# tsdconseil/libtsd

Measured on AMD Instinct MI355X. Metric: Msamples/s, 127-tap FIR on 2^26 cfloat stream, higher is better.
Workload: dtype f32 (complex64 data, real f32 taps); 1 GPU; configs[1]: 127-tap FIR (design_rif_fen lp 0.02, real taps via filtrer()) on 2^26-sample Veccf per GPU, inputs resident in HBM; method=overlap-save, samples_per_gpu=67108864, pre_warm_steps=150, backend=none (one process, one GPU), world_size=1, self_launched=False

## Files before the change

### libtsd_amd/csrc/ols.hip

```cpp
#include "fir_internal.hpp"
#include "fft1024_wave.hpp"
#include <cstdlib>

namespace tsdgpu {

using namespace w1024;
constexpr int OLS_N = 1024;
#ifndef OLS_SCALAR
#define OLS_SCALAR 1
#endif
#ifndef OLS_RUN_DEFAULT
#define OLS_RUN_DEFAULT 2
#endif
#ifndef OLS_DYN_DEFAULT
#define OLS_DYN_DEFAULT 16
#endif
constexpr int OLS_MAX_CTR = 32;
#if OLS_SCALAR
using cv = cpx;
#else
using cv = v2f;
#endif
__device__ __forceinline__ cv mkv(float a, float b) { return Make<cv>::of(a, b); }

constexpr bool NT = false;
__device__ __forceinline__ cv ntload(const cv *p)
{
  v2f t = __builtin_nontemporal_load(reinterpret_cast<const v2f *>(p));
  return mkv(t.x, t.y);
}
__device__ __forceinline__ void ntstore(cv *p, cv v)
{
  v2f t = {v.x, v.y};
  __builtin_nontemporal_store(t, reinterpret_cast<v2f *>(p));
}
template <bool EDGE>
__device__ __forceinline__ void ols_fetch_real(cv (&v)[16], const float *__restrict__ x, const float *__restrict__ hist,
                                               int histlen, int Km1, int L, int64_t n, int64_t b, int lane)
{
  const int64_t ga = 2 * b * (int64_t) L - Km1, gb = ga + L;
  if (!EDGE) {
    const float *xa = x + ga, *xb = x + gb;
#pragma unroll
    for (int r = 0; r < 16; r++) v[r] = mkv(xa[64 * r + lane], xb[64 * r + lane]);
  } else {
#pragma unroll
    for (int r = 0; r < 16; r++) {
      const int64_t g1 = ga + 64 * r + lane, g2 = gb + 64 * r + lane;
      v[r] = mkv(g1 < 0 ? hist[histlen + g1] : (g1 < n ? x[g1] : 0.f), g2 < 0 ? hist[histlen + g2] : (g2 < n ? x[g2] : 0.f));
    }
  }
}
template <bool EDGE>
__device__ __forceinline__ void ols_fetch(cv (&v)[16], const cv *__restrict__ x, const cv *__restrict__ hist,
                                          int histlen, int Km1, int L, int64_t n, int64_t b, int lane)
{
  const int64_t g0 = b * (int64_t) L - Km1;
  if (!EDGE) {
    const cv *xb = x + g0;
#pragma unroll
    for (int r = 0; r < 16; r++) v[r] = NT ? ntload(xb + 64 * r + lane) : xb[64 * r + lane];
  } else {
#pragma unroll
    for (int r = 0; r < 16; r++) {
      const int64_t g = g0 + 64 * r + lane;
      v[r] = g < 0 ? hist[histlen + g] : (g < n ? x[g] : mkv(0.f, 0.f));
    }
  }
}

struct OlsDyn {
  unsigned *ctr;
  unsigned base, Q;
  int NC;
  int64_t nunits;
};
struct RegTab {
  cv v[16];
  __device__ __forceinline__ const cv &operator[](int r) const { return v[r]; }
};

template <bool EDGE, bool REAL, int R0, bool DYN>
__device__ __forceinline__ void ols_body(cv *lds, const void *__restrict__ xv, const void *__restrict__ histv,
                                         void *__restrict__ yv, const cv *__restrict__ Hreg,
                                         const cv *__restrict__ TW1, const cv *__restrict__ TW2, int Km1,
                                         int histlen, int L, int64_t n, int64_t b_lo, int64_t b_hi, int64_t G,
                                         int64_t w, int64_t cgrp, int R, OlsDyn dyn)
{
  const int lane = threadIdx.x & 63;
  const cv *x = (const cv *) xv, *hist = (const cv *) histv;
  cv *y = (cv *) yv;
  const float *xr = (const float *) xv, *histr = (const float *) histv;
  float *yr = (float *) yv;
  RegTab tw1r, tw2r, Hr;
#pragma unroll
  for (int r = 0; r < 16; r++) {
    tw1r.v[r] = TW1[r * 64 + lane];
    tw2r.v[r] = TW2[r * 64 + lane];
    Hr.v[r] = Hreg[r * 64 + lane];
  }
  auto sync = []() {
    __builtin_amdgcn_fence(__ATOMIC_RELEASE, "wavefront");
    __builtin_amdgcn_wave_barrier();
    __builtin_amdgcn_fence(__ATOMIC_ACQUIRE, "wavefront");
  };

  const int64_t slot = (G % 8 == 0) ? (w % 8) * (G / 8) + w / 8 : w;
  const int ctr_c = DYN ? (int) (cgrp % dyn.NC) : 0;
  auto pull_issue = [&]() -> unsigned {
    unsigned v = 0;
    if (lane == 0) v = __hip_atomic_fetch_add(dyn.ctr + ctr_c * 32, 1u, __ATOMIC_RELAXED, __HIP_MEMORY_SCOPE_AGENT);
    return v;
  };
  auto pull = [&]() -> int64_t {
    for (;;) {
      const unsigned v = (unsigned) __builtin_amdgcn_readfirstlane((int) pull_issue()) - dyn.base;
      if (v >= dyn.Q) return -1;
      const int64_t u = (int64_t) v * dyn.NC + ctr_c;
      if (u < dyn.nunits) return u;
    }
  };
  auto pull_finish = [&](unsigned raw) -> int64_t {
    const unsigned v = (unsigned) __builtin_amdgcn_readfirstlane((int) raw) - dyn.base;
    if (v >= dyn.Q) return -1;
    const int64_t u = (int64_t) v * dyn.NC + ctr_c;
    return u < dyn.nunits ? u : pull();
  };
  int64_t unit = EDGE ? 0 : (DYN ? pull() : slot);
  if (unit < 0) return;
  int64_t run0 = EDGE ? b_lo : b_lo + unit * R;
  int64_t b = run0;
  if (b >= b_hi) return;

  int64_t pulled = -1;
  auto process = [&](cv (&cur)[16], cv (&nxt)[16], int64_t blk, int64_t nb, bool inrun) {
    const bool more = !EDGE && nb < b_hi;
    cv keep[R0 > 0 ? R0 : 1], pre[R0 > 0 ? R0 : 1];
#pragma unroll
    for (int r = 0; r < R0; r++) keep[r] = cur[(16 - R0 + r) & 15];
    const int64_t pb = more ? nb : blk;
    if (!EDGE && R0 > 0) {
      if (!REAL) {
        const cv *xb = x + (pb * (int64_t) L - Km1);
        if (!inrun) {
#pragma unroll
          for (int r = 0; r < R0; r++) pre[r] = xb[64 * r + lane];
        }
#pragma unroll
        for (int r = R0; r < 16; r++) nxt[r] = NT ? ntload(xb + 64 * r + lane) : xb[64 * r + lane];
      } else {
        const float *xa = xr + (2 * pb * (int64_t) L - Km1), *xb = xa + L;
        if (!inrun) {
#pragma unroll
          for (int r = 0; r < R0; r++) pre[r] = mkv(xa[64 * r + lane], xb[64 * r + lane]);
        }
#pragma unroll
        for (int r = R0; r < 16; r++) nxt[r] = mkv(xa[64 * r + lane], xb[64 * r + lane]);
      }
    } else if (!EDGE) {
      if (REAL) ols_fetch_real<EDGE>(nxt, xr, histr, histlen, Km1, L, n, pb, lane);
      else ols_fetch<EDGE>(nxt, x, hist, histlen, Km1, L, n, pb, lane);
    }
    const bool pulls = DYN && more && !inrun;
    unsigned raw = 0;
    if (pulls) raw = pull_issue();
    forward(cur, lds, lane, tw1r, tw2r, sync);
#pragma unroll
    for (int r = 0; r < 16; r++) cur[r] = cmul(cur[r], Hr[r]);
    inverse(cur, lds, lane, tw1r, tw2r, sync);
    sync();
    if (!EDGE) {
#pragma unroll
      for (int r = R0; r < 16; r++) asm volatile("" ::"v"(nxt[r]));
#pragma unroll
      for (int r = 0; r < R0; r++) {
        asm volatile("" : "+v"(keep[r]));
        if (inrun) nxt[r] = REAL ? mkv(keep[r].y, nxt[(16 - R0 + r) & 15].x) : keep[r];
        else nxt[r] = pre[r];
      }
    }
    if (pulls) pulled = pull_finish(raw);
    const int r0 = (!EDGE && R0 > 0) ? R0 : Km1 >> 6;
    if (!REAL) {
      const int64_t o0 = blk * (int64_t) L;
      cv *yb = y + (o0 - Km1);
#pragma unroll
      for (int r = 0; r < 16; r++) {
        const int t = 64 * r + lane;
        if (!EDGE) {
          if (r >= r0) { if (NT) ntstore(yb + t, cur[r]); else yb[t] = cur[r]; }
        } else {
          if (r >= r0 && o0 + t - Km1 < n) yb[t] = cur[r];
        }
      }
    } else {
      const int64_t oa = 2 * blk * (int64_t) L, ob = oa + L;
      float *ya = yr + (oa - Km1), *yb = yr + (ob - Km1);
#pragma unroll
      for (int r = 0; r < 16; r++) {
        const int t = 64 * r + lane;
        if (!EDGE) {
          if (r >= r0) { ya[t] = cur[r].x; yb[t] = cur[r].y; }
        } else {
          if (r >= r0 && oa + t - Km1 < n) ya[t] = cur[r].x;
          if (r >= r0 && ob + t - Km1 < n) yb[t] = cur[r].y;
        }
      }
    }
  };

  cv A[16], B[16];
  if (REAL) ols_fetch_real<EDGE>(A, xr, histr, histlen, Km1, L, n, b, lane);
  else ols_fetch<EDGE>(A, x, hist, histlen, Km1, L, n, b, lane);
  if (EDGE) {
    process(A, B, b, b_hi, false);
    return;
  }
#pragma unroll
  for (int r = 0; r < 16; r++) asm volatile("" ::"v"(A[r]));
  int i = 0;
  constexpr int64_t END = INT64_MAX;
  auto unit_after = [&](int64_t u) -> int64_t {
    if (DYN) return pulled;
    return b_lo + (u + G) * R < b_hi ? u + G : -1;
  };
  int64_t unit_next = DYN ? pull() : unit_after(unit);
  auto next_of = [&](int64_t &nb, bool &inrun) {
    inrun = i + 1 < R && b + 1 < b_hi;
    nb = inrun ? b + 1 : (unit_next >= 0 ? b_lo + unit_next * R : END);
  };
  auto advance = [&](int64_t nb, bool inrun) {
    if (inrun) i++;
    else {
      i = 0;
      run0 = nb;
      unit = unit_next;
      unit_next = unit_after(unit);
    }
    b = nb;
  };
  for (;;) {
    int64_t nb;
    bool inrun;
    next_of(nb, inrun);
    process(A, B, b, nb, inrun);
    if (nb >= b_hi) break;
    advance(nb, inrun);
    next_of(nb, inrun);
    process(B, A, b, nb, inrun);
    if (nb >= b_hi) break;
    advance(nb, inrun);
  }
}

template <bool REAL, int R0, bool DYN>
__global__ __launch_bounds__(64, 2) void ols_kernel(const void *__restrict__ x, const void *__restrict__ hist,
                                                    void *__restrict__ hist_next, void *__restrict__ y,
                                                    const cpx *__restrict__ Hreg, const cpx *__restrict__ TW1,
                                                    const cpx *__restrict__ TW2, int Km1, int histlen, int L,
                                                    int64_t n, int64_t b_lo, int64_t b_hi, int64_t nblocks, int G,
                                                    int ne, int64_t n_lo, int64_t b_tail, int R, OlsDyn dyn)
{
  __shared__ cv lds[LDS_ELEMS];
  const int64_t w = (int64_t) blockIdx.x;
  const int lane = threadIdx.x & 63;
  if (w < G) {
    ols_body<false, REAL, R0, DYN>(lds, x, hist, y, (const cv *) Hreg, (const cv *) TW1, (const cv *) TW2, Km1, histlen, L, n, b_lo, b_hi, G,
                                       w, (int64_t) blockIdx.x / 8, R, dyn);
  } else if (w < G + ne) {
    const int64_t b = (w - G) < n_lo ? (int64_t) (w - G) : b_tail + (w - G - n_lo);
    ols_body<true, REAL, 0, false>(lds, x, hist, y, (const cv *) Hreg, (const cv *) TW1, (const cv *) TW2, Km1, histlen, L, n, b, nblocks, 1, 0, 0, 1, dyn);
  } else if (w == G + ne) {
    for (int i = lane; i < histlen; i += 64) {
      const int64_t g = n - histlen + i;
      if (REAL) ((float *) hist_next)[i] = g < 0 ? ((const float *) hist)[histlen + g] : ((const float *) x)[g];
      else ((cpx *) hist_next)[i] = g < 0 ? ((const cpx *) hist)[histlen + g] : ((const cpx *) x)[g];
    }
  }
}

bool ols_preferred(const tsdgpu_fir *f)
{
  if (ols_long_supported(f)) return true;
  if (f->data_type == TSDGPU_C64) return f->K >= (f->tap_type == TSDGPU_F32 ? 57 : 48) && f->K <= 513;
  return f->tap_type == TSDGPU_F32 && f->K >= 40 && f->K <= 513;
}

int ols_plan_create(tsdgpu_fir *f)
{
  if (ols_long_supported(f)) return ols_long_plan_create(f);
  if (f->K > OLS_N - 63) {
    f->method = TSDGPU_FIR_DIRECT;
    return TSDGPU_OK;
  }
  const int N = OLS_N, K = f->K;
  f->ols_N = N;
  f->ols_L = N - (int) (cdiv(K - 1, 64) * 64);
  std::vector<double> hr(K), hi(K, 0.0);
  if (f->tap_type == TSDGPU_F32) {
    const float *t = (const float *) f->taps_host.data();
    for (int i = 0; i < K; i++) hr[i] = t[i];
  } else {
    const float *t = (const float *) f->taps_host.data();
    for (int i = 0; i < K; i++) { hr[i] = t[2 * i]; hi[i] = t[2 * i + 1]; }
  }
  struct Tables {
    std::vector<double> c, s;
    std::vector<cpx> tw12;
    Tables() : c(OLS_N / 2), s(OLS_N / 2), tw12(2 * OLS_N)
    {
      const double PI = 3.14159265358979323846;
      for (int i = 0; i < OLS_N / 2; i++) { c[i] = std::cos(2 * PI * i / OLS_N); s[i] = -std::sin(2 * PI * i / OLS_N); }
      fill_twiddles(tw12.data(), tw12.data() + OLS_N);
    }
  };
  static const Tables *tb = new Tables();
  std::vector<double> ar(N, 0.0), ai(N, 0.0);
  int logn = 0;
  while ((1 << logn) < N) logn++;
  for (int i = 0; i < K; i++) {
    int rv = 0;
    for (int b = 0; b < logn; b++) rv |= ((i >> b) & 1) << (logn - 1 - b);
    ar[rv] = hr[i];
    ai[rv] = hi[i];
  }
  for (int len = 2; len <= N; len <<= 1) {
    const int half = len / 2, step = N / len;
    for (int base = 0; base < N; base += len)
      for (int j = 0; j < half; j++) {
        const double wr = tb->c[(size_t) j * step], wi = tb->s[(size_t) j * step];
        const int a = base + j, b = a + half;
        const double tr = ar[b] * wr - ai[b] * wi, ti = ar[b] * wi + ai[b] * wr;
        ar[b] = ar[a] - tr; ai[b] = ai[a] - ti;
        ar[a] += tr; ai[a] += ti;
      }
  }
  std::vector<cpx> img(3 * (size_t) N);
  for (int lane = 0; lane < 64; lane++)
    for (int r = 0; r < 16; r++) {
      const int k = freq_index(lane, r);
      img[r * 64 + lane] = mk((float) (ar[k] / N), (float) (ai[k] / N));
    }
  std::copy(tb->tw12.begin(), tb->tw12.end(), img.begin() + N);
  const size_t bytes = (size_t) N * sizeof(cpx);
  const size_t ctr_bytes = (size_t) OLS_MAX_CTR * 128;
  img.resize(3 * (size_t) N + ctr_bytes / sizeof(cpx), mk(0.f, 0.f));
  if (hipMalloc(&f->d_H, 3 * bytes + ctr_bytes) != hipSuccess)
    return set_err(TSDGPU_ERR_HIP, "ols: hipMalloc failed: %s", hipGetErrorString(hipGetLastError()));
  if (hipMemcpy(f->d_H, img.data(), 3 * bytes + ctr_bytes, hipMemcpyHostToDevice) != hipSuccess)
    return set_err(TSDGPU_ERR_HIP, "ols: upload failed: %s", hipGetErrorString(hipGetLastError()));
  f->d_ctr = (unsigned *) ((char *) f->d_H + 3 * bytes);
  f->ctr_base = 0;
  static const std::pair<int, int> occ = []() {
    int dev = 0, cus = 256, per_cu = 8;
    (void) hipGetDevice(&dev);
    (void) hipDeviceGetAttribute(&cus, hipDeviceAttributeMultiprocessorCount, dev);
    if (hipOccupancyMaxActiveBlocksPerMultiprocessor(&per_cu, ols_kernel<false, 2, true>, 64, 0) != hipSuccess || per_cu < 1) {
      (void) hipGetLastError();
      per_cu = 8;
    }
    return std::make_pair(cus, per_cu);
  }();
  const int cus = occ.first, per_cu = occ.second;
  f->ols_grid = cus * per_cu;
  if (getenv("TSDGPU_DEBUG")) fprintf(stderr, "[tsdgpu] ols plan: N=%d K=%d L=%d cus=%d waves/CU=%d grid=%d waves\n", N, K, f->ols_L, cus, per_cu, f->ols_grid);
  return TSDGPU_OK;
}

void ols_plan_destroy(tsdgpu_fir *f)
{
  if (f->d_H) (void) hipFree(f->d_H);
  f->d_H = nullptr;
  f->d_ctr = nullptr;
}

int ols_step(tsdgpu_fir *f, const void *x, void *y, int64_t n, hipStream_t st)
{
  const bool real = f->data_type == TSDGPU_F32;
  const int L = f->ols_L;
  const int64_t LB = real ? 2 * (int64_t) L : L;
  const int64_t nblocks = cdiv(n, LB);
  const cpx *d = (const cpx *) f->d_H;
  const int64_t ovl = OLS_N - L;
  const int64_t b_lo = std::min<int64_t>(nblocks, f->K > 1 ? cdiv(ovl, LB) : 0);
  const int64_t b_hi = std::max<int64_t>(b_lo, n / LB);
  int64_t grid = 0;
  const int r0 = (int) (ovl / 64);
  const char *run_s = dev_switch("OLS_RUN");
  const int run_env = run_s ? atoi(run_s) : OLS_RUN_DEFAULT;
  const char *nc_s = dev_switch("OLS_DYN");
  int NC = nc_s ? atoi(nc_s) : OLS_DYN_DEFAULT;
  if (NC < 0 || NC > OLS_MAX_CTR || f->capturable || !f->d_ctr || stream_is_capturing(st)) NC = 0;
  int R = 1;
  unsigned ctr_add = 0;
  OlsDyn dyn = {f->d_ctr, f->ctr_base, 0u, NC > 0 ? NC : 1, 0};
  if (b_hi > b_lo) {
    const int64_t nint = b_hi - b_lo;
    if (r0 >= 1 && r0 <= 4 && run_env > 1 && nint >= (int64_t) f->ols_grid * run_env * 2) R = run_env;
    const int64_t nruns = cdiv(nint, R);
    const char *min_s = dev_switch("OLS_DYN_MIN");
    const int64_t dyn_min = min_s ? atoi(min_s) : 4;
    if (NC > 0 && nruns >= dyn_min * (int64_t) f->ols_grid) {
      const int64_t grp = (int64_t) 8 * NC;
      grid = std::max<int64_t>(grp, (f->ols_grid / grp) * grp);
      if (NC != f->ctr_nc) {
        TSD_HIP(hipMemsetAsync(f->d_ctr, 0, (size_t) OLS_MAX_CTR * 128, st));
        f->ctr_base = 0;
        f->ctr_nc = NC;
        dyn.base = 0;
      }
      dyn.nunits = nruns;
      dyn.Q = (unsigned) cdiv(nruns, NC);
      ctr_add = dyn.Q + (unsigned) (grid / NC);
    } else {
      NC = 0;
      grid = nruns < f->ols_grid ? nruns : f->ols_grid;
      if (nruns > grid) {
        const int64_t rounds = cdiv(nruns, grid);
        grid = cdiv(cdiv(nruns, rounds), 8) * 8;
      }
    }
  } else NC = 0;
  const int64_t b_lo_w = b_lo;
  const int64_t n_lo = b_lo, b_tail = b_hi;
  const int ne = (int) (n_lo + (nblocks - b_tail));
  int64_t e[2] = {n_lo, b_tail};
  const int nxt = f->cur ^ 1;
  const unsigned nwg = (unsigned) (grid + ne + 1);
#define OLS_LAUNCH(REAL, R0, DYN)                                                                                                     \
  hipLaunchKernelGGL((ols_kernel<REAL, R0, DYN>), dim3(nwg), dim3(64), 0, st, x, (const void *) fir_hist_read(f),                        \
                     f->hist[nxt], y, d, d + OLS_N, d + 2 * OLS_N, OLS_N - L, f->HL, L, n, b_lo_w, b_hi, nblocks, (int) grid, ne,   \
                     e[0], e[1], R, dyn)
#define OLS_LAUNCH_R0(REAL, DYN)                                        \
  switch (R > 1 ? r0 : 0) {                                             \
    case 1: OLS_LAUNCH(REAL, 1, DYN); break;                            \
    case 2: OLS_LAUNCH(REAL, 2, DYN); break;                            \
    case 3: OLS_LAUNCH(REAL, 3, DYN); break;                            \
    case 4: OLS_LAUNCH(REAL, 4, DYN); break;                            \
    default: OLS_LAUNCH(REAL, 0, DYN); break;                           \
  }
  if (real) {
    if (NC > 0) { OLS_LAUNCH_R0(true, true) } else { OLS_LAUNCH_R0(true, false) }
  } else {
    if (NC > 0) { OLS_LAUNCH_R0(false, true) } else { OLS_LAUNCH_R0(false, false) }
  }
#undef OLS_LAUNCH_R0
#undef OLS_LAUNCH
  if (const hipError_t le = hipGetLastError(); le != hipSuccess) {
    if (NC > 0) f->ctr_nc = 0;
    return set_err(TSDGPU_ERR_HIP, "fir_step: overlap-save launch failed: %s", hipGetErrorString(le));
  }
  f->ctr_base += ctr_add;
  f->cur = nxt;
  return TSDGPU_OK;
}

__global__ __launch_bounds__(64, 2) void ola1024_kernel(const cpx *__restrict__ x, cpx *__restrict__ y, const cpx *__restrict__ Hreg,
                                                        const cpx *__restrict__ TW1, const cpx *__restrict__ TW2,
                                                        const cpx *__restrict__ svg_in, cpx *__restrict__ svg_out, int64_t B, int per)
{
  __shared__ cv lds[LDS_ELEMS];
  const int lane = threadIdx.x;
  const int64_t b_lo = (int64_t) blockIdx.x * per, b_hi = min(B, b_lo + (int64_t) per);
  if (b_lo >= B) return;
  cv tw1[16], tw2[16], H[16];
#pragma unroll
  for (int r = 0; r < 16; r++) {
    tw1[r] = ((const cv *) TW1)[r * 64 + lane];
    tw2[r] = ((const cv *) TW2)[r * 64 + lane];
    H[r] = ((const cv *) Hreg)[r * 64 + lane];
  }
  auto sync = []() {
    __builtin_amdgcn_fence(__ATOMIC_RELEASE, "wavefront");
    __builtin_amdgcn_wave_barrier();
    __builtin_amdgcn_fence(__ATOMIC_ACQUIRE, "wavefront");
  };
  const cv *xs = (const cv *) x;
  cv *ys = (cv *) y;
  cv cur[16], carry[8], nxt[8];
  auto transform = [&](cv (&v)[16]) {
    forward(v, lds, lane, tw1, tw2, sync);
#pragma unroll
    for (int r = 0; r < 16; r++) v[r] = cmul(v[r], H[r]);
    inverse(v, lds, lane, tw1, tw2, sync);
    sync();
  };
  if (b_lo == 0) {
#pragma unroll
    for (int r = 0; r < 8; r++) carry[r] = ((const cv *) svg_in)[64 * r + lane];
  } else {
#pragma unroll
    for (int r = 0; r < 8; r++) { cur[r] = mkv(0.f, 0.f); cur[8 + r] = xs[(b_lo - 1) * 512 + 64 * r + lane]; }
    transform(cur);
#pragma unroll
    for (int r = 0; r < 8; r++) carry[r] = cur[8 + r];
  }
#pragma unroll
  for (int r = 0; r < 8; r++) nxt[r] = xs[b_lo * 512 + 64 * r + lane];
  for (int64_t b = b_lo; b < b_hi; b++) {
#pragma unroll
    for (int r = 0; r < 8; r++) { cur[r] = mkv(0.f, 0.f); cur[8 + r] = nxt[r]; }
    const bool more = b + 1 < b_hi;
    if (more) {
#pragma unroll
      for (int r = 0; r < 8; r++) nxt[r] = xs[(b + 1) * 512 + 64 * r + lane];
    }
    transform(cur);
    if (more) {
#pragma unroll
      for (int r = 0; r < 8; r++) asm volatile("" ::"v"(nxt[r]));
    }
#pragma unroll
    for (int r = 0; r < 8; r++) {
      ys[b * 512 + 64 * r + lane] = mkv(cur[r].x + carry[r].x, cur[r].y + carry[r].y);
      carry[r] = cur[8 + r];
    }
  }
  if (b_hi == B) {
#pragma unroll
    for (int r = 0; r < 8; r++) ((cv *) svg_out)[64 * r + lane] = carry[r];
  }
}

void ola1024_tables(const cpx *H_host, cpx *out3)
{
  for (int lane = 0; lane < 64; lane++)
    for (int r = 0; r < 16; r++) {
      const cpx h = H_host[freq_index(lane, r)];
      out3[r * 64 + lane] = mk(h.x / 1024.f, h.y / 1024.f);
    }
  fill_twiddles(out3 + 1024, out3 + 2048);
}

int ola1024_launch(const cpx *x, cpx *y, const cpx *tables3, const cpx *svg_in, cpx *svg_out, int64_t B, hipStream_t st)
{
  if (B <= 0) return TSDGPU_OK;
  const int per = (int) std::min<int64_t>(16, std::max<int64_t>(1, cdiv(B, 2048)));
  const int64_t grid = cdiv(B, per);
  if (grid > 0x7fffffff) return set_err(TSDGPU_ERR_UNSUPPORTED, "ola: too many blocks in one call");
  hipLaunchKernelGGL(ola1024_kernel, dim3((unsigned) grid), dim3(64), 0, st, x, y, tables3, tables3 + 1024, tables3 + 2048, svg_in, svg_out, B, per);
  TSD_HIP(hipGetLastError());
  return TSDGPU_OK;
}

__global__ __launch_bounds__(64, 2) void olaw512_kernel(const cpx *__restrict__ blk0, int nrest, const cpx *__restrict__ x, cpx *__restrict__ y,
                                                        const cpx *__restrict__ Hreg, const cpx *__restrict__ TW1, const cpx *__restrict__ TW2,
                                                        const float *__restrict__ fen, const cpx *__restrict__ svg_in,
                                                        const cpx *__restrict__ last_in, const cpx *__restrict__ prev_half_in,
                                                        cpx *__restrict__ svg_out, cpx *__restrict__ last_out, int64_t B, int per,
                                                        int skip_first)
{
  __shared__ cv lds[LDS_ELEMS];
  const int lane = threadIdx.x;
  const int64_t b_lo = (int64_t) blockIdx.x * per, b_hi = min(B, b_lo + (int64_t) per);
  if (b_lo >= B) return;
  const int sig = (lane >> 1) & 1, c = 2 * (lane >> 2) + (lane & 1);
  cv tw1[16], tw2[16], H[8];
  float win[16];
#pragma unroll
  for (int r = 0; r < 16; r++) {
    tw1[r] = ((const cv *) TW1)[r * 64 + lane];
    tw2[r] = ((const cv *) TW2)[r * 64 + lane];
    win[r] = fen[32 * r + c];
  }
#pragma unroll
  for (int q = 0; q < 8; q++) H[q] = ((const cv *) Hreg)[q * 64 + lane];
  auto sync = []() {
    __builtin_amdgcn_fence(__ATOMIC_RELEASE, "wavefront");
    __builtin_amdgcn_wave_barrier();
    __builtin_amdgcn_fence(__ATOMIC_ACQUIRE, "wavefront");
  };
  auto sample = [&](int64_t i) -> cv {
    if (i < 0) return ((const cv *) prev_half_in)[i + 256];
    if (i < 512) return ((const cv *) blk0)[i];
    return ((const cv *) x)[i - nrest];
  };
  auto xchg = [&](cv a) -> cv {
    return mkv(__shfl_xor(a.x, 2), __shfl_xor(a.y, 2));
  };
  cv v[16], keep[8];
  int64_t p = b_lo <= 1 ? 0 : b_lo - 2;
  if (b_lo <= 1) {
#pragma unroll
    for (int r = 0; r < 8; r++) keep[r] = ((const cv *) svg_in)[256 + 32 * r + c];
    if (b_lo == 0 && !skip_first) {
#pragma unroll
      for (int r = 0; r < 8; r++) {
        const int i = 32 * r + c;
        cv o = ((const cv *) last_in)[256 * sig + i];
        if (sig) {
          const cv g = ((const cv *) svg_in)[i];
          o = mkv(o.x + g.x * 0.5f, o.y + g.y * 0.5f);
        }
        ((cv *) y)[256 * sig + i] = o;
      }
    }
  } else {
#pragma unroll
    for (int r = 0; r < 8; r++) keep[r] = mkv(0.f, 0.f);
  }
  const int64_t p_end = b_hi == B ? B : b_hi - 1;
  for (; p < p_end; p++) {
    const int64_t base = 512 * p - 256 + 256 * sig;
#pragma unroll
    for (int r = 0; r < 16; r++) {
      const cv a = sample(base + 32 * r + c);
      v[r] = mkv(a.x * win[r], a.y * win[r]);
    }
    forward_pair512(v, lds, lane, tw1, tw2, sync);
#pragma unroll
    for (int r = 0; r < 16; r++) v[r] = cmul(v[r], H[2 * (r >> 2) + (r & 1)]);
    inverse_pair512(v, lds, lane, tw1, tw2, sync);
    sync();
    cv got[8];
#pragma unroll
    for (int r = 0; r < 8; r++) got[r] = xchg(v[8 + r]);
    if (p + 1 < B) {
      if (p + 1 >= b_lo) {
        cv *yo = (cv *) y + (p + 1 - skip_first) * 512 + 256 * sig + c;
#pragma unroll
        for (int r = 0; r < 8; r++) {
          const cv o = sig ? got[r] : keep[r];
          yo[32 * r] = mkv(o.x * 0.5f + v[r].x * 0.5f, o.y * 0.5f + v[r].y * 0.5f);
        }
      }
    } else {
      if (sig) {
#pragma unroll
        for (int r = 0; r < 16; r++) ((cv *) svg_out)[32 * r + c] = v[r];
      } else {
#pragma unroll
        for (int r = 0; r < 8; r++) {
          ((cv *) last_out)[32 * r + c] = mkv(keep[r].x * 0.5f + v[r].x * 0.5f, keep[r].y * 0.5f + v[r].y * 0.5f);
          ((cv *) last_out)[256 + 32 * r + c] = mkv(v[8 + r].x * 0.5f, v[8 + r].y * 0.5f);
        }
      }
    }
#pragma unroll
    for (int r = 0; r < 8; r++) keep[r] = got[r];
  }
}

void olaw512_tables(const cpx *H_host, cpx *out)
{
  for (int lane = 0; lane < 64; lane++)
    for (int q = 0; q < 8; q++) {
      const cpx h = H_host[pair512_freq_index(lane, 4 * (q >> 1) + (q & 1))];
      out[q * 64 + lane] = mk(h.x / 512.f, h.y / 512.f);
    }
  fill_twiddles_pair512(out + 512, out + 512 + 1024);
}

int olaw512_launch(const cpx *blk0, int nrest, const cpx *x, cpx *y, const cpx *tables, const float *fen, const cpx *svg_in, const cpx *last_in,
                   const cpx *prev_half_in, cpx *svg_out, cpx *last_out, int64_t B, int skip_first, hipStream_t st)
{
  if (B <= 0) return TSDGPU_OK;
  const int per = (int) std::min<int64_t>(16, std::max<int64_t>(2, cdiv(B, 2048)));
  const int64_t grid = cdiv(B, per);
  if (grid > 0x7fffffff) return set_err(TSDGPU_ERR_UNSUPPORTED, "ola: too many blocks in one call");
  hipLaunchKernelGGL(olaw512_kernel, dim3((unsigned) grid), dim3(64), 0, st, blk0, nrest, x, y, tables, tables + 512, tables + 512 + 1024, fen, svg_in,
                     last_in, prev_half_in, svg_out, last_out, B, per, skip_first);
  TSD_HIP(hipGetLastError());
  return TSDGPU_OK;
}

__global__ __launch_bounds__(64, 2) void welch1024_kernel(const cpx *__restrict__ x, const float *__restrict__ w,
                                                          const cpx *__restrict__ TW1, const cpx *__restrict__ TW2,
                                                          float *__restrict__ part, int64_t nseg, int per)
{
  __shared__ cv lds[LDS_ELEMS];
  const int lane = threadIdx.x;
  const int64_t k_lo = (int64_t) blockIdx.x * per, k_hi = min(nseg, k_lo + (int64_t) per);
  cv tw1[16], tw2[16];
  float win[16], acc[16];
#pragma unroll
  for (int r = 0; r < 16; r++) {
    tw1[r] = ((const cv *) TW1)[r * 64 + lane];
    tw2[r] = ((const cv *) TW2)[r * 64 + lane];
    win[r] = w[64 * r + lane];
    acc[r] = 0.f;
  }
  auto sync = []() {
    __builtin_amdgcn_fence(__ATOMIC_RELEASE, "wavefront");
    __builtin_amdgcn_wave_barrier();
    __builtin_amdgcn_fence(__ATOMIC_ACQUIRE, "wavefront");
  };
  const cv *xs = (const cv *) x;
  cv cur[16], nxt[16];
  if (k_lo < k_hi) {
#pragma unroll
    for (int r = 0; r < 16; r++) nxt[r] = xs[k_lo * 512 + 64 * r + lane];
  }
  for (int64_t k = k_lo; k < k_hi; k++) {
#pragma unroll
    for (int r = 0; r < 16; r++) cur[r] = mkv(nxt[r].x * win[r], nxt[r].y * win[r]);
    if (k + 1 < k_hi) {
#pragma unroll
      for (int r = 0; r < 16; r++) nxt[r] = xs[(k + 1) * 512 + 64 * r + lane];
    }
    forward(cur, lds, lane, tw1, tw2, sync);
    sync();
#pragma unroll
    for (int r = 0; r < 16; r++) acc[r] += cur[r].x * cur[r].x + cur[r].y * cur[r].y;
  }
#pragma unroll
  for (int r = 0; r < 16; r++) part[(size_t) blockIdx.x * 1024 + ((freq_index(lane, r) + 512) & 1023)] = acc[r] * (1.0f / 1024.0f);
}

int welch1024_launch(const cpx *x, const float *w, const cpx *tw2x1024, float *part, int64_t nseg, int per, hipStream_t st)
{
  const int64_t grid = cdiv(nseg, per);
  hipLaunchKernelGGL(welch1024_kernel, dim3((unsigned) grid), dim3(64), 0, st, x, w, tw2x1024, tw2x1024 + 1024, part, nseg, per);
  TSD_HIP(hipGetLastError());
  return TSDGPU_OK;
}

void welch1024_tables(cpx *out2) { fill_twiddles(out2, out2 + 1024); }

}
```

Baseline: 335,000 Msamples/s.

## Give dynamic OLS workers static first units and fold edge work into them

In the dynamic-scheduling path, each worker now takes its first two units statically (slot and slot+G) and only pulls from the atomic counter after that. The counter range is shifted by 2G, and a dummy increment is issued when a worker skips its pulls so the counter accounting stays balanced. Edge blocks and the history copy are no longer handled by extra workgroups; the first ne workers process them before their main loop, so the grid shrinks to exactly the dynamic grid size. The first input block fetch is moved ahead of the twiddle and filter register loads to overlap latency. Optional wall-clock stamp instrumentation is added behind a compile flag.

```diff
diff --git a/libtsd_amd/csrc/ols.hip b/libtsd_amd/csrc/ols.hip
--- a/libtsd_amd/csrc/ols.hip
+++ b/libtsd_amd/csrc/ols.hip
@@ -16,6 +16,19 @@
 #define OLS_DYN_DEFAULT 16
 #endif
 constexpr int OLS_MAX_CTR = 32;
+#ifndef OLS_STAMPS
+#define OLS_STAMPS 0
+#endif
+#if OLS_STAMPS
+enum { ST_ENTRY, ST_UNIT, ST_LANDED, ST_STORE0, ST_STORE1, ST_EXIT, ST_ROLE, ST_ITEM, ST_N };
+struct OlsClk { unsigned long long t[ST_N]; };
+#define OLS_STAMP(clk, i) ((clk).t[i] = wall_clock64())
+static unsigned long long *g_stamp_buf = nullptr;
+static int64_t g_stamp_cap = 0;
+#else
+struct OlsClk {};
+#define OLS_STAMP(clk, i) ((void) 0)
+#endif
 #if OLS_SCALAR
 using cv = cpx;
 #else
@@ -74,6 +87,9 @@
   unsigned base, Q;
   int NC;
   int64_t nunits;
+#if OLS_STAMPS
+  unsigned long long *stamps;
+#endif
 };
 struct RegTab {
   cv v[16];
@@ -85,7 +101,7 @@
                                          void *__restrict__ yv, const cv *__restrict__ Hreg,
                                          const cv *__restrict__ TW1, const cv *__restrict__ TW2, int Km1,
                                          int histlen, int L, int64_t n, int64_t b_lo, int64_t b_hi, int64_t G,
-                                         int64_t w, int64_t cgrp, int R, OlsDyn dyn)
+                                         int64_t w, int64_t cgrp, int R, OlsDyn dyn, OlsClk &clk)
 {
   const int lane = threadIdx.x & 63;
   const cv *x = (const cv *) xv, *hist = (const cv *) histv;
@@ -93,12 +109,6 @@
   const float *xr = (const float *) xv, *histr = (const float *) histv;
   float *yr = (float *) yv;
   RegTab tw1r, tw2r, Hr;
-#pragma unroll
-  for (int r = 0; r < 16; r++) {
-    tw1r.v[r] = TW1[r * 64 + lane];
-    tw2r.v[r] = TW2[r * 64 + lane];
-    Hr.v[r] = Hreg[r * 64 + lane];
-  }
   auto sync = []() {
     __builtin_amdgcn_fence(__ATOMIC_RELEASE, "wavefront");
     __builtin_amdgcn_wave_barrier();
@@ -117,20 +127,35 @@
       const unsigned v = (unsigned) __builtin_amdgcn_readfirstlane((int) pull_issue()) - dyn.base;
       if (v >= dyn.Q) return -1;
       const int64_t u = (int64_t) v * dyn.NC + ctr_c;
-      if (u < dyn.nunits) return u;
+      if (u < dyn.nunits) return 2 * G + u;
     }
   };
   auto pull_finish = [&](unsigned raw) -> int64_t {
     const unsigned v = (unsigned) __builtin_amdgcn_readfirstlane((int) raw) - dyn.base;
     if (v >= dyn.Q) return -1;
     const int64_t u = (int64_t) v * dyn.NC + ctr_c;
-    return u < dyn.nunits ? u : pull();
-  };
-  int64_t unit = EDGE ? 0 : (DYN ? pull() : slot);
-  if (unit < 0) return;
+    return u < dyn.nunits ? 2 * G + u : pull();
+  };
+  auto pull_fail = [&]() {
+    if (lane == 0) (void) __hip_atomic_fetch_add(dyn.ctr + ctr_c * 32, 1u, __ATOMIC_RELAXED, __HIP_MEMORY_SCOPE_AGENT);
+  };
+  int64_t unit = EDGE ? 0 : slot;
+  OLS_STAMP(clk, ST_UNIT);
   int64_t run0 = EDGE ? b_lo : b_lo + unit * R;
   int64_t b = run0;
-  if (b >= b_hi) return;
+  if (b >= b_hi) {
+    if (DYN) pull_fail();
+    return;
+  }
+  cv A[16], B[16];
+  if (REAL) ols_fetch_real<EDGE>(A, xr, histr, histlen, Km1, L, n, b, lane);
+  else ols_fetch<EDGE>(A, x, hist, histlen, Km1, L, n, b, lane);
+#pragma unroll
+  for (int r = 0; r < 16; r++) {
+    tw1r.v[r] = TW1[r * 64 + lane];
+    tw2r.v[r] = TW2[r * 64 + lane];
+    Hr.v[r] = Hreg[r * 64 + lane];
+  }
 
   int64_t pulled = -1;
   auto process = [&](cv (&cur)[16], cv (&nxt)[16], int64_t blk, int64_t nb, bool inrun) {
@@ -207,24 +232,31 @@
         }
       }
     }
-  };
-
-  cv A[16], B[16];
-  if (REAL) ols_fetch_real<EDGE>(A, xr, histr, histlen, Km1, L, n, b, lane);
-  else ols_fetch<EDGE>(A, x, hist, histlen, Km1, L, n, b, lane);
+#if OLS_STAMPS
+    if (!clk.t[ST_STORE0]) OLS_STAMP(clk, ST_STORE0);
+    OLS_STAMP(clk, ST_STORE1);
+#endif
+  };
+
   if (EDGE) {
     process(A, B, b, b_hi, false);
     return;
   }
 #pragma unroll
-  for (int r = 0; r < 16; r++) asm volatile("" ::"v"(A[r]));
+  for (int r = 0; r < 16; r++) {
+    asm volatile("" ::"v"(A[r]));
+    asm volatile("" ::"v"(tw1r.v[r]), "v"(tw2r.v[r]), "v"(Hr.v[r]));
+  }
+#if OLS_STAMPS
+  asm volatile("s_waitcnt vmcnt(0)" ::: "memory");
+  OLS_STAMP(clk, ST_LANDED);
+#endif
   int i = 0;
   constexpr int64_t END = INT64_MAX;
-  auto unit_after = [&](int64_t u) -> int64_t {
-    if (DYN) return pulled;
-    return b_lo + (u + G) * R < b_hi ? u + G : -1;
-  };
-  int64_t unit_next = DYN ? pull() : unit_after(unit);
+  auto static_after = [&](int64_t u) -> int64_t { return b_lo + (u + G) * R < b_hi ? u + G : -1; };
+  auto unit_after = [&](int64_t u) -> int64_t { return DYN ? pulled : static_after(u); };
+  int64_t unit_next = static_after(unit);
+  if (DYN && unit_next < 0) pull_fail();
   auto next_of = [&](int64_t &nb, bool &inrun) {
     inrun = i + 1 < R && b + 1 < b_hi;
     nb = inrun ? b + 1 : (unit_next >= 0 ? b_lo + unit_next * R : END);
@@ -264,20 +296,53 @@
   __shared__ cv lds[LDS_ELEMS];
   const int64_t w = (int64_t) blockIdx.x;
   const int lane = threadIdx.x & 63;
-  if (w < G) {
-    ols_body<false, REAL, R0, DYN>(lds, x, hist, y, (const cv *) Hreg, (const cv *) TW1, (const cv *) TW2, Km1, histlen, L, n, b_lo, b_hi, G,
-                                       w, (int64_t) blockIdx.x / 8, R, dyn);
-  } else if (w < G + ne) {
-    const int64_t b = (w - G) < n_lo ? (int64_t) (w - G) : b_tail + (w - G - n_lo);
-    ols_body<true, REAL, 0, false>(lds, x, hist, y, (const cv *) Hreg, (const cv *) TW1, (const cv *) TW2, Km1, histlen, L, n, b, nblocks, 1, 0, 0, 1, dyn);
-  } else if (w == G + ne) {
+  OlsClk clk;
+#if OLS_STAMPS
+  for (int i = 0; i < ST_N; i++) clk.t[i] = 0;
+  OLS_STAMP(clk, ST_ENTRY);
+  clk.t[ST_ROLE] = DYN ? (w < ne ? 1 : (w == ne ? 2 : 0)) : (w < G ? 0 : (w < G + ne ? 1 : 2));
+#endif
+  auto edge_item = [&](int64_t e) {
+    const int64_t b = e < n_lo ? e : b_tail + (e - n_lo);
+    OlsClk iclk = {};
+    ols_body<true, REAL, 0, false>(lds, x, hist, y, (const cv *) Hreg, (const cv *) TW1, (const cv *) TW2, Km1, histlen, L, n, b, nblocks, 1, 0, 0, 1, dyn, iclk);
+  };
+  auto history_item = [&]() {
     for (int i = lane; i < histlen; i += 64) {
       const int64_t g = n - histlen + i;
       if (REAL) ((float *) hist_next)[i] = g < 0 ? ((const float *) hist)[histlen + g] : ((const float *) x)[g];
       else ((cpx *) hist_next)[i] = g < 0 ? ((const cpx *) hist)[histlen + g] : ((const cpx *) x)[g];
     }
-  }
-}
+  };
+  if (DYN) {
+    if (w < ne) edge_item(w);
+    else if (w == ne) history_item();
+    if (w <= ne) OLS_STAMP(clk, ST_ITEM);
+    ols_body<false, REAL, R0, DYN>(lds, x, hist, y, (const cv *) Hreg, (const cv *) TW1, (const cv *) TW2, Km1, histlen, L, n, b_lo, b_hi, G,
+                                       w, (int64_t) blockIdx.x / 8, R, dyn, clk);
+  } else if (w < G) {
+    ols_body<false, REAL, R0, DYN>(lds, x, hist, y, (const cv *) Hreg, (const cv *) TW1, (const cv *) TW2, Km1, histlen, L, n, b_lo, b_hi, G,
+                                       w, (int64_t) blockIdx.x / 8, R, dyn, clk);
+  } else if (w < G + ne) {
+    edge_item(w - G);
+  } else if (w == G + ne) {
+    history_item();
+  }
+#if OLS_STAMPS
+  if (!DYN && w >= G) OLS_STAMP(clk, ST_ITEM);
+  OLS_STAMP(clk, ST_EXIT);
+  if (dyn.stamps && lane == 0)
+    for (int i = 0; i < ST_N; i++) dyn.stamps[(int64_t) blockIdx.x * ST_N + i] = clk.t[i];
+#endif
+}
+
+#if OLS_STAMPS
+extern "C" void tsdgpu_ols_stamp_buffer(void *buf, int64_t cap)
+{
+  g_stamp_buf = (unsigned long long *) buf;
+  g_stamp_cap = cap;
+}
+#endif
 
 bool ols_preferred(const tsdgpu_fir *f)
 {
@@ -400,17 +465,19 @@
     const int64_t nruns = cdiv(nint, R);
     const char *min_s = dev_switch("OLS_DYN_MIN");
     const int64_t dyn_min = min_s ? atoi(min_s) : 4;
-    if (NC > 0 && nruns >= dyn_min * (int64_t) f->ols_grid) {
-      const int64_t grp = (int64_t) 8 * NC;
-      grid = std::max<int64_t>(grp, (f->ols_grid / grp) * grp);
+    const int64_t grp = (int64_t) 8 * std::max(NC, 1);
+    const int64_t dgrid = std::max<int64_t>(grp, (f->ols_grid / grp) * grp);
+    const int64_t n_edge = b_lo + (nblocks - b_hi);
+    if (NC > 0 && nruns >= dyn_min * (int64_t) f->ols_grid && dgrid > n_edge) {
+      grid = dgrid;
       if (NC != f->ctr_nc) {
         TSD_HIP(hipMemsetAsync(f->d_ctr, 0, (size_t) OLS_MAX_CTR * 128, st));
         f->ctr_base = 0;
         f->ctr_nc = NC;
         dyn.base = 0;
       }
-      dyn.nunits = nruns;
-      dyn.Q = (unsigned) cdiv(nruns, NC);
+      dyn.nunits = std::max<int64_t>(0, nruns - 2 * grid);
+      dyn.Q = (unsigned) cdiv(dyn.nunits, NC);
       ctr_add = dyn.Q + (unsigned) (grid / NC);
     } else {
       NC = 0;
@@ -426,7 +493,10 @@
   const int ne = (int) (n_lo + (nblocks - b_tail));
   int64_t e[2] = {n_lo, b_tail};
   const int nxt = f->cur ^ 1;
-  const unsigned nwg = (unsigned) (grid + ne + 1);
+  const unsigned nwg = NC > 0 ? (unsigned) grid : (unsigned) (grid + ne + 1);
+#if OLS_STAMPS
+  dyn.stamps = (int64_t) nwg <= g_stamp_cap ? g_stamp_buf : nullptr;
+#endif
 #define OLS_LAUNCH(REAL, R0, DYN)                                                                                                     \
   hipLaunchKernelGGL((ols_kernel<REAL, R0, DYN>), dim3(nwg), dim3(64), 0, st, x, (const void *) fir_hist_read(f),                        \
                      f->hist[nxt], y, d, d + OLS_N, d + 2 * OLS_N, OLS_N - L, f->HL, L, n, b_lo_w, b_hi, nblocks, (int) grid, ne,   \
```

Result: no change. 333,800 Msamples/s (-0.4%).
